# jameshensman/pyvb

Measured on AMD Instinct MI355X. Metric: VB update iterations/sec (T=10k, D=64, N=1024 LDS); ELBO rel-err vs NumPy, higher is better.
Workload: dtype f64; 1 GPU; LDS T=10000 D=64 K=64, 1024 replicates per GPU (BASELINE configs[2]); replicates_total=1024, parallelism=replicates sharded over 1 GPU(s), collective=none (1 GPU), degraded=False

## Files before the change

### pyvb_amd/csrc/k_sweep.hip

```cpp
#include "common.h"

struct SweepArgs {
    const double* Xold; double* Xnew; const double* Y; const double* gains; const int* warm;
    const double *A_mean, *C_mean;
    const double *QA, *RC;
    double* trash;
    double* U;
    double* Sxx;
    int N, T, D, K, dir;
    int W;
    const unsigned char* active;
    const int* len;
    int keep_x;
    Layout L;
};

#define MFMA(a, b, c) __builtin_amdgcn_mfma_f64_16x16x4f64((a), (b), (c), 0, 0, 0)

constexpr int BOUNDARY_BLOCK = 16;

template <int NP>
__device__ __forceinline__ double boundary_chain(double v, const double* M, size_t stride, size_t off, int n, const double* u) {
#pragma unroll
    for (int b = 0; b < NP; b += BOUNDARY_BLOCK) {
        if (b >= n) break;
        double m[BOUNDARY_BLOCK];
#pragma unroll
        for (int e = 0; e < BOUNDARY_BLOCK; ++e) m[e] = M[(size_t)(b + e < n ? b + e : n - 1) * stride + off];
#pragma unroll
        for (int e = 0; e < BOUNDARY_BLOCK; ++e) v += (b + e < n ? m[e] : 0.0) * u[b + e];
    }
    return v;
}

template <int DP, int KP>
__device__ __forceinline__ double boundary_update(bool first, const double* g, const Layout& L, const double* Am, const double* Cm,
                                                  int D, int K, int lane, double xn, const double* y, double* ux, double* uy, double* vs,
                                                  const double* QA = nullptr, const double* RC = nullptr) {
    const bool dense = QA != nullptr;
    const int lc = lane < D ? lane : D - 1, kc = lane < K ? lane : K - 1;
    const double qb = g[L.oqr + lc], rb = g[L.oqr + 64 + kc], yk = y[kc], w0 = g[L.ow0 + lc];
    ux[lane] = lane < D ? ((first && !dense) ? qb * xn : xn) : 0.0;
    uy[lane] = lane < K ? (dense ? yk : rb * yk) : 0.0;
    __syncthreads();
    double v = boundary_chain<DP>(first ? w0 : 0.0, dense ? QA : Am, first ? D : 1, (size_t)lc * (first ? 1 : D), D, ux);
    if (!first && !dense) v = qb * v;
    v = boundary_chain<KP>(v, dense ? RC : Cm, D, lc, K, uy);
    vs[lane] = lane < D ? v : 0.0;
    __syncthreads();
    const double s = boundary_chain<DP>(0.0, g + (first ? L.oS0 : L.oS2), L.DP, lc, D, vs);
    __syncthreads();
    return lane < D ? s : 0.0;
}

template <int DT, int KT, bool FULL, int MODE, bool SPLIT>
__global__ void __launch_bounds__(64) k_sweep(SweepArgs a) {
    constexpr int DS = 4 * DT, KS = 4 * KT, DP = 16 * DT, KP = 16 * KT;
    __shared__ double gl[MODE == 2 ? DP * 17 : DT * KS * 64];
    __shared__ double xs[64];
    __shared__ double vs[64], ux[64], uy[64];
    const int n = blockIdx.x, w = SPLIT ? blockIdx.y : 0, lane = threadIdx.x, c = lane & 15, q = lane >> 4;
    if (!a.active[n]) return;
    const int T = a.T, D = a.D, K = a.K;
    const int TL = a.len ? a.len[n] : T;
    const bool fwd = (a.dir == 0);
    const int sgn = fwd ? 1 : -1;
    const Layout& L = a.L;
    const double* g = a.gains + (size_t)n * L.gains_total;
    const double* Xo = a.Xold + (size_t)n * T * DP;
    double* Xn = a.Xnew + (size_t)n * T * DP;
    const double* Yn = a.Y + (size_t)n * T * K;

    double rn[DT][DS], ip[DT][DS];
    {
        const double* Rn = g + (fwd ? L.oFn : L.oBn);
        const double* Ip = g + (fwd ? L.oBn : L.oFn);
#pragma unroll
        for (int m = 0; m < DT; ++m)
#pragma unroll
            for (int s = 0; s < DS; ++s) {
                rn[m][s] = Rn[(m * DS + s) * 64 + lane];
                ip[m][s] = (MODE == 2) ? 0.0 : Ip[(m * DS + s) * 64 + lane];
            }
        if constexpr (MODE != 2) {
            const double* Gp = g + L.oGp;
            for (int i = 0; i < DT * KS; ++i) gl[i * 64 + lane] = Gp[i * 64 + lane];
        }
    }

    const int Tint = TL - 2;
    const int Lw = SPLIT ? split_part_len(T, a.W) : Tint;
    const int ow = SPLIT ? w * Lw : 0;
    const int Tw = (Tint - ow < Lw) ? Tint - ow : Lw;
    const int J = a.warm[n * 2 + a.dir];

    const int t_first = fwd ? 0 : TL - 1, t_last = fwd ? TL - 1 : 0;
    const double* Am = a.A_mean + (size_t)n * D * D;
    const double* Cm = a.C_mean + (size_t)n * K * D;
    const double* QAm = a.QA ? a.QA + (size_t)n * D * D : nullptr;
    const double* RCm = a.RC ? a.RC + (size_t)n * K * D : nullptr;
    if (!SPLIT || ow <= J) {
        const double* xo = Xo + (size_t)(t_first + sgn) * DP;
        const double s = boundary_update<DP, KP>(fwd, g, L, Am, Cm, D, K, lane, xo[xpos(lane < D ? lane : D - 1)],
                                                 Yn + (size_t)t_first * K, ux, uy, vs, QAm, RCm);
        if (w == 0 && lane < DP) Xn[(size_t)t_first * DP + xpos(lane)] = (lane < D) ? s : 0.0;
        xs[lane] = (lane < D) ? s : 0.0;
    }
    __builtin_amdgcn_fence(__ATOMIC_RELEASE, "workgroup");
    __builtin_amdgcn_s_barrier();
    __builtin_amdgcn_fence(__ATOMIC_ACQUIRE, "workgroup");

    if (Tw > 0) {
        const int Lseg = (Tw + 15) >> 4;
        const int cL = c * Lseg;
        const int before = ow + cL;
        const int jc = -(J < before ? J : before);
        const int jstart = -((J < ow + 15 * Lseg) ? J : ow + 15 * Lseg);
        d4 x[DT];
#pragma unroll
        for (int m = 0; m < DT; ++m)
#pragma unroll
            for (int r = 0; r < 4; ++r) x[m][r] = (jc == -before) ? xs[16 * m + 4 * r + q] : 0.0;

        const int tbase = fwd ? (1 + before) : (TL - 2 - before);
        const int tsafe = fwd ? 1 : TL - 2;
        auto active = [&](int j) { int tt = cL + j; return j >= jc && j < Lseg && tt < Tw; };
        d2 yv[KS / 2];
        d4 mo[DT];
        auto load_y = [&](int j, d2* dst) {
            const double* p = Yn + (size_t)(active(j) ? tbase + sgn * j : tsafe) * K;
#pragma unroll
            for (int i = 0; i < KS / 2; ++i) {
                const int d0 = 8 * i + 2 * q;
                if constexpr (FULL) {
                    dst[i] = *reinterpret_cast<const d2*>(p + d0);
                } else {
                    dst[i][0] = p[d0 < K ? d0 : K - 1];
                    dst[i][1] = p[d0 + 1 < K ? d0 + 1 : K - 1];
                }
            }
        };
        auto load_o = [&](int j, d4* dst) {
            const double* p = Xo + (size_t)((active(j) ? tbase + sgn * j : tsafe) + sgn) * DP;
#pragma unroll
            for (int m = 0; m < DT; ++m) dst[m] = *reinterpret_cast<const d4*>(p + (m * 4 + q) * 4);
        };
        auto store_x = [&](double* out) {
#pragma unroll
            for (int m = 0; m < DT; ++m) *reinterpret_cast<d4*>(out + (m * 4 + q) * 4) = x[m];
        };
        double* const trash = a.trash + (size_t)n * 256;
        double* out_pending = trash;
        double* const Un = a.U + (size_t)n * T * DP;
        auto u_row = [&](int j) { return (active(j) && j >= 0) ? Un + (size_t)(tbase + sgn * j) * DP : trash; };
        auto load_u = [&](int j, d4* dst) {
            const double* p = Un + (size_t)(active(j) ? tbase + sgn * j : tsafe) * DP;
#pragma unroll
            for (int m = 0; m < DT; ++m) dst[m] = *reinterpret_cast<const d4*>(p + (m * 4 + q) * 4);
        };
        auto select_tile = [&](int m, bool act, const d4* acc) {
#pragma unroll
            for (int r = 0; r < 4; ++r) x[m][r] = act ? acc[m][r] : x[m][r];
        };
        auto pending_row = [&](int j, bool act) {
            return (act && j >= 0 && (a.keep_x || before + j == Tint - 1)) ? Xn + (size_t)(tbase + sgn * j) * DP : trash;
        };
        auto finish_step = [&](int j, const d4* acc) {
            const bool act = active(j);
#pragma unroll
            for (int m = 0; m < DT; ++m) select_tile(m, act, acc);
            out_pending = pending_row(j, act);
        };
        auto mul_resident = [&](d4* acc, auto& M, const d4* v) {
#pragma unroll
            for (int s = 0; s < DS; ++s)
#pragma unroll
                for (int m = 0; m < DT; ++m) acc[m] = MFMA(M[m][s], v[s >> 2][s & 3], acc[m]);
        };
        if constexpr (MODE == 2) {
            constexpr int PF = 3;
            d4 ub[PF][DT];
            double* const tl = gl;
            for (int i = lane; i < DP * 17; i += 64) tl[i] = 0.0;
            d4 sxx[DT][DT];
#pragma unroll
            for (int m = 0; m < DT; ++m)
#pragma unroll
                for (int k = 0; k < DT; ++k) sxx[m][k] = d4{0.0, 0.0, 0.0, 0.0};
            auto tile_read = [&](double (*xt)[4]) {
#pragma unroll
                for (int m = 0; m < DT; ++m)
#pragma unroll
                    for (int s4 = 0; s4 < 4; ++s4) xt[m][s4] = tl[(16 * m + c) * 17 + 4 * s4 + q];
            };
            auto tile_accumulate = [&](double (*xt)[4]) {
#pragma unroll
                for (int s4 = 0; s4 < 4; ++s4)
#pragma unroll
                    for (int m = 0; m < DT; ++m)
#pragma unroll
                        for (int k = m; k < DT; ++k) sxx[m][k] = MFMA(xt[m][s4], xt[k][s4], sxx[m][k]);
            };
            auto tile_stage = [&](int m, bool keep) {
#pragma unroll
                for (int r = 0; r < 4; ++r) tl[(16 * m + 4 * r + q) * 17 + c] = keep ? x[m][r] : 0.0;
            };
#pragma unroll
            for (int p = 0; p < PF; ++p) { load_u(jstart + p, ub[p]); store_x(trash + 64 * p); }
            for (int j = jstart; j < Lseg; j += PF) {
#pragma unroll
                for (int p = 0; p < PF; ++p) {
                    d4 acc[DT];
                    double xt[DT][4];
                    tile_read(xt);
#pragma unroll
                    for (int m = 0; m < DT; ++m) acc[m] = ub[p][m];
                    __builtin_amdgcn_sched_barrier(0);
                    load_u(j + p + PF, ub[p]);
                    store_x(out_pending);
                    __builtin_amdgcn_sched_barrier(0);
                    mul_resident(acc, rn, x);
                    const bool act = active(j + p);
                    const bool keep = act && j + p >= 0;
                    tile_accumulate(xt);
                    finish_step(j + p, acc);
#pragma unroll
                    for (int m = 0; m < DT; ++m) tile_stage(m, keep);
                }
            }
            {
                double xt[DT][4];
                tile_read(xt);
                tile_accumulate(xt);
            }
            store_x(out_pending);
            double* Sn = a.Sxx + ((size_t)n * (SPLIT ? a.W : 1) + w) * DP * DP;
#pragma unroll
            for (int m = 0; m < DT; ++m)
#pragma unroll
                for (int k = m; k < DT; ++k)
#pragma unroll
                    for (int e = 0; e < 4; ++e) {
                        const int row = 16 * m + 4 * e + q, col = 16 * k + c;
                        Sn[(size_t)row * DP + col] = sxx[m][k][e];
                        if (k > m) Sn[(size_t)col * DP + row] = sxx[m][k][e];
                    }
        } else {
        load_y(jstart, yv);
        store_x(trash);
        if constexpr (MODE == 1) store_x(trash + 64);
        load_o(jstart, mo);
        for (int j = jstart; j < Lseg; ++j) {
            d4 acc[DT];
            {
#pragma unroll
                for (int m = 0; m < DT; ++m) acc[m] = d4{0.0, 0.0, 0.0, 0.0};
                int goff = lane;
                asm volatile("" : "+v"(goff));
#pragma unroll
                for (int s = 0; s < KS; ++s)
#pragma unroll
                    for (int m = 0; m < DT; ++m) acc[m] = MFMA(gl[(m * KS + s) * 64 + goff], yv[s >> 1][s & 1], acc[m]);
                __builtin_amdgcn_sched_barrier(0);
                load_y(j + 1, yv);
                store_x(out_pending);
                __builtin_amdgcn_sched_barrier(0);
            }
            mul_resident(acc, rn, x);
            {
                if constexpr (MODE == 1) {
                    __builtin_amdgcn_sched_barrier(0);
                    double* ur = u_row(j);
#pragma unroll
                    for (int m = 0; m < DT; ++m) *reinterpret_cast<d4*>(ur + (m * 4 + q) * 4) = acc[m];
                    __builtin_amdgcn_sched_barrier(0);
                }
                mul_resident(acc, ip, mo);
                __builtin_amdgcn_sched_barrier(0);
                load_o(j + 1, mo);
                __builtin_amdgcn_sched_barrier(0);
            }
            finish_step(j, acc);
        }
        store_x(out_pending);
        }
        const int clast = (Tw - 1) / Lseg;
        __builtin_amdgcn_s_barrier();
        if (c == clast) {
#pragma unroll
            for (int m = 0; m < DT; ++m)
#pragma unroll
                for (int r = 0; r < 4; ++r) xs[16 * m + 4 * r + q] = x[m][r];
        }
        __builtin_amdgcn_fence(__ATOMIC_RELEASE, "workgroup");
        __builtin_amdgcn_s_barrier();
        __builtin_amdgcn_fence(__ATOMIC_ACQUIRE, "workgroup");
    }

    if (!SPLIT || w == ((Tint > 0) ? (Tint - 1) / Lw : 0)) {
        const double s = boundary_update<DP, KP>(!fwd, g, L, Am, Cm, D, K, lane, xs[lane],
                                                 Yn + (size_t)t_last * K, ux, uy, vs, QAm, RCm);
        if (lane < DP) Xn[(size_t)t_last * DP + xpos(lane)] = (lane < D) ? s : 0.0;
    }
}

struct StepArgs {
    double* X; const double* Y; const double* gains; const double *A_mean, *C_mean, *QA, *RC;
    const unsigned char* active;
    const int* len;
    int N, T, D, K, t;
    Layout L;
};

__global__ void __launch_bounds__(64) k_step(StepArgs a) {
    const int n = blockIdx.x, lane = threadIdx.x;
    if (!a.active[n]) return;
    const int T = a.T, D = a.D, K = a.K, t = a.t, DP = a.L.DP;
    const int TL = a.len ? a.len[n] : T;
    if (t >= TL) return;
    const Layout& L = a.L;
    const double* g = a.gains + (size_t)n * L.gains_total;
    double* X = a.X + (size_t)n * T * DP;
    const double* y = a.Y + ((size_t)n * T + t) * K;
    const int cls = (t == 0) ? 0 : (t == TL - 1 ? 2 : 1);
    const int row = lane % DP;
    if (cls != 1) {
        __shared__ double vs[64], ux[64], uy[64];
        const double* nbr = X + (size_t)(cls == 0 ? 1 : TL - 2) * DP;
        const double s = boundary_update<64, 64>(cls == 0, g, L, a.A_mean + (size_t)n * D * D, a.C_mean + (size_t)n * K * D, D, K, lane,
                                                 nbr[xpos(lane < D ? lane : D - 1)], y, ux, uy, vs,
                                                 a.QA ? a.QA + (size_t)n * D * D : nullptr, a.RC ? a.RC + (size_t)n * K * D : nullptr);
        if (lane < DP) X[(size_t)t * DP + xpos(lane)] = (lane < D) ? s : 0.0;
        return;
    }
    const int DS = L.DS, KS = L.KS;
    double s = 0.0;
    for (int j = 0; j < D; ++j) s += g[L.oFn + pos_nat(row, j, DS)] * X[(size_t)(t - 1) * DP + xpos(j)];
    for (int j = 0; j < D; ++j) s += g[L.oBn + pos_nat(row, j, DS)] * X[(size_t)(t + 1) * DP + xpos(j)];
    for (int k = 0; k < K; ++k) s += g[L.oGp + pos_perm(row, k, KS)] * y[k];
    if (lane < DP) X[(size_t)t * DP + xpos(lane)] = (lane < D) ? s : 0.0;
}

template <int DT, int KT>
static int launch_sweep_t(pyvb_lds* h, const SweepArgs& a, bool read_cache) {
    const bool full = h->D == 16 * DT && a.K == 16 * KT;
    const int mode = a.dir == PYVB_FORWARD ? 1 : (read_cache ? 2 : 0);
#define PYVB_SWEEP_CASE(F, M) do { if (h->W > 1) hipLaunchKernelGGL((k_sweep<DT, KT, F, M, true>), dim3(h->N, h->W), dim3(64), 0, h->stream, a); \
                                   else hipLaunchKernelGGL((k_sweep<DT, KT, F, M, false>), dim3(h->N), dim3(64), 0, h->stream, a); } while (0)
    if (full) { if (mode == 1) PYVB_SWEEP_CASE(true, 1); else if (mode == 2) PYVB_SWEEP_CASE(true, 2); else PYVB_SWEEP_CASE(true, 0); }
    else { if (mode == 1) PYVB_SWEEP_CASE(false, 1); else if (mode == 2) PYVB_SWEEP_CASE(false, 2); else PYVB_SWEEP_CASE(false, 0); }
#undef PYVB_SWEEP_CASE
    return PYVB_OK;
}

int launch_sweep(pyvb_lds* h, int direction, int src, bool read_cache, bool keep_x) {
    if (h->big) return launch_sweep_big(h, direction, src, read_cache);
    SweepArgs a;
    a.keep_x = (keep_x || direction != PYVB_FORWARD) ? 1 : 0;
    a.W = h->W;
    a.Xold = h->X[src]; a.Xnew = h->X[1 - src]; a.Y = lds_sweep_Y(h); a.gains = h->gains; a.warm = h->warm;
    a.trash = h->trash; a.U = h->U; a.Sxx = h->sxx; a.A_mean = h->A_mean; a.C_mean = lds_sweep_C(h);
    a.QA = h->dense ? h->QA : nullptr; a.RC = h->dense ? h->RC : nullptr;
    a.N = h->N; a.T = h->T; a.D = h->D; a.K = lds_sweep_K(h); a.dir = direction; a.L = h->L; a.active = h->active; a.len = h->len;
    {
        TimedLaunch tl(h, direction == PYVB_FORWARD ? PYVB_K_SWEEP_FWD : PYVB_K_SWEEP_BWD);
        switch (h->L.DT * 10 + h->L.KT) {
            case 11: launch_sweep_t<1, 1>(h, a, read_cache); break;
            case 12: launch_sweep_t<1, 2>(h, a, read_cache); break;
            case 14: launch_sweep_t<1, 4>(h, a, read_cache); break;
            case 21: launch_sweep_t<2, 1>(h, a, read_cache); break;
            case 22: launch_sweep_t<2, 2>(h, a, read_cache); break;
            case 24: launch_sweep_t<2, 4>(h, a, read_cache); break;
            case 41: launch_sweep_t<4, 1>(h, a, read_cache); break;
            case 42: launch_sweep_t<4, 2>(h, a, read_cache); break;
            case 44: launch_sweep_t<4, 4>(h, a, read_cache); break;
            default: pyvb_set_error("unsupported tile shape"); return PYVB_E_ARG;
        }
    }
    HIPCHK(hipGetLastError());
    return PYVB_OK;
}

struct PermArgs { const double* src; double* dst; size_t rows; int D, DP, to_internal; };
__global__ void __launch_bounds__(256) k_permute(PermArgs a) {
    const int per = a.DP > 64 ? 128 : 64;
    const size_t row = (size_t)blockIdx.x * (256 / per) + (threadIdx.x / per);
    const int d = threadIdx.x % per;
    if (row >= a.rows || d >= a.DP) return;
    if (a.to_internal) a.dst[row * a.DP + xpos(d)] = (d < a.D) ? a.src[row * a.D + d] : 0.0;
    else if (d < a.D) a.dst[row * a.D + d] = a.src[row * a.DP + xpos(d)];
}

int launch_permute(pyvb_lds* h, const double* src, double* dst, int to_internal) {
    PermArgs a; a.src = src; a.dst = dst; a.rows = (size_t)h->N * h->T; a.D = h->D; a.DP = h->L.DP; a.to_internal = to_internal;
    const size_t per_block = a.DP > 64 ? 2 : 4;
    hipLaunchKernelGGL(k_permute, dim3((unsigned)((a.rows + per_block - 1) / per_block)), dim3(256), 0, h->stream, a);
    HIPCHK(hipGetLastError());
    return PYVB_OK;
}

struct CarryArgs { const double* src; double* dst; const unsigned char* active; size_t per; };
__global__ void __launch_bounds__(256) k_carry(CarryArgs a) {
    const int n = blockIdx.y;
    if (a.active[n]) return;
    const double* s = a.src + (size_t)n * a.per;
    double* d = a.dst + (size_t)n * a.per;
    for (size_t i = (size_t)blockIdx.x * 256 + threadIdx.x; i < a.per; i += (size_t)gridDim.x * 256) d[i] = s[i];
}

int launch_carry(pyvb_lds* h, const double* src, double* dst, size_t per) {
    CarryArgs a; a.src = src; a.dst = dst; a.active = h->active; a.per = per;
    const size_t blocks = (per + 255) / 256;
    hipLaunchKernelGGL(k_carry, dim3((unsigned)(blocks < 64 ? blocks : 64), h->N), dim3(256), 0, h->stream, a);
    HIPCHK(hipGetLastError());
    return PYVB_OK;
}

int launch_step(pyvb_lds* h, int t) {
    if (h->big) return launch_step_big(h, t);
    StepArgs a;
    a.X = h->X[h->st.cur]; a.Y = lds_sweep_Y(h); a.gains = h->gains; a.A_mean = h->A_mean; a.C_mean = lds_sweep_C(h);
    a.QA = h->dense ? h->QA : nullptr; a.RC = h->dense ? h->RC : nullptr;
    a.N = h->N; a.T = h->T; a.D = h->D; a.K = lds_sweep_K(h); a.t = t; a.L = h->L; a.active = h->active; a.len = h->len;
    TimedLaunch tl(h, PYVB_K_STEP);
    hipLaunchKernelGGL(k_step, dim3(h->N), dim3(64), 0, h->stream, a);
    HIPCHK(hipGetLastError());
    return PYVB_OK;
}
```

Measured before the change: 92.15 VB iterations/s per 1024 replicates (whole job).

## Replace forward-sweep warm-up with seam correction pass and specialize keep_x

```diff
diff --git a/pyvb_amd/csrc/k_sweep.hip b/pyvb_amd/csrc/k_sweep.hip
--- a/pyvb_amd/csrc/k_sweep.hip
+++ b/pyvb_amd/csrc/k_sweep.hip
@@ -1,4 +1,6 @@
+#include <type_traits>
 #include "common.h"
+#include "sweep_plan.h"
 
 struct SweepArgs {
     const double* Xold; double* Xnew; const double* Y; const double* gains; const int* warm;
@@ -53,7 +55,7 @@
     return lane < D ? s : 0.0;
 }
 
-template <int DT, int KT, bool FULL, int MODE, bool SPLIT>
+template <int DT, int KT, bool FULL, int MODE, bool SPLIT, bool KEEPX = true>
 __global__ void __launch_bounds__(64) k_sweep(SweepArgs a) {
     constexpr int DS = 4 * DT, KS = 4 * KT, DP = 16 * DT, KP = 16 * KT;
     __shared__ double gl[MODE == 2 ? DP * 17 : DT * KS * 64];
@@ -88,11 +90,12 @@
         }
     }
 
-    const int Tint = TL - 2;
+    const int J = a.warm[n * 2 + a.dir];
+    const SweepPart part = sweep_part(TL, T, SPLIT ? a.W : 1, w, J, MODE == 1 && fwd);
+    const int Tint = part.Tint;
     const int Lw = SPLIT ? split_part_len(T, a.W) : Tint;
-    const int ow = SPLIT ? w * Lw : 0;
-    const int Tw = (Tint - ow < Lw) ? Tint - ow : Lw;
-    const int J = a.warm[n * 2 + a.dir];
+    const int ow = part.ow;
+    const int Tw = part.Tw;
 
     const int t_first = fwd ? 0 : TL - 1, t_last = fwd ? TL - 1 : 0;
     const double* Am = a.A_mean + (size_t)n * D * D;
@@ -111,20 +114,19 @@
     __builtin_amdgcn_fence(__ATOMIC_ACQUIRE, "workgroup");
 
     if (Tw > 0) {
-        const int Lseg = (Tw + 15) >> 4;
-        const int cL = c * Lseg;
-        const int before = ow + cL;
-        const int jc = -(J < before ? J : before);
-        const int jstart = -((J < ow + 15 * Lseg) ? J : ow + 15 * Lseg);
+        const int Lseg = part.Lseg;
+        const SweepColumn col = sweep_column(part, c);
+        const int before = col.before;
+        const int jstart = sweep_first_step(part);
         d4 x[DT];
 #pragma unroll
         for (int m = 0; m < DT; ++m)
 #pragma unroll
-            for (int r = 0; r < 4; ++r) x[m][r] = (jc == -before) ? xs[16 * m + 4 * r + q] : 0.0;
+            for (int r = 0; r < 4; ++r) x[m][r] = (col.kind == SWEEP_START_BOUNDARY) ? xs[16 * m + 4 * r + q] : 0.0;
 
         const int tbase = fwd ? (1 + before) : (TL - 2 - before);
         const int tsafe = fwd ? 1 : TL - 2;
-        auto active = [&](int j) { int tt = cL + j; return j >= jc && j < Lseg && tt < Tw; };
+        auto active = [&](int j) { return sweep_active(part, col, j); };
         d2 yv[KS / 2];
         d4 mo[DT];
         auto load_y = [&](int j, d2* dst) {
@@ -163,7 +165,7 @@
             for (int r = 0; r < 4; ++r) x[m][r] = act ? acc[m][r] : x[m][r];
         };
         auto pending_row = [&](int j, bool act) {
-            return (act && j >= 0 && (a.keep_x || before + j == Tint - 1)) ? Xn + (size_t)(tbase + sgn * j) * DP : trash;
+            return (act && j >= 0 && (KEEPX || before + j == Tint - 1)) ? Xn + (size_t)(tbase + sgn * j) * DP : trash;
         };
         auto finish_step = [&](int j, const d4* acc) {
             const bool act = active(j);
@@ -207,26 +209,35 @@
             };
 #pragma unroll
             for (int p = 0; p < PF; ++p) { load_u(jstart + p, ub[p]); store_x(trash + 64 * p); }
-            for (int j = jstart; j < Lseg; j += PF) {
-#pragma unroll
-                for (int p = 0; p < PF; ++p) {
-                    d4 acc[DT];
-                    double xt[DT][4];
-                    tile_read(xt);
-#pragma unroll
-                    for (int m = 0; m < DT; ++m) acc[m] = ub[p][m];
-                    __builtin_amdgcn_sched_barrier(0);
-                    load_u(j + p + PF, ub[p]);
-                    store_x(out_pending);
-                    __builtin_amdgcn_sched_barrier(0);
-                    mul_resident(acc, rn, x);
-                    const bool act = active(j + p);
-                    const bool keep = act && j + p >= 0;
-                    tile_accumulate(xt);
-                    finish_step(j + p, acc);
+            auto step = [&](int j, int p, d4* ubp, auto counted) {
+                constexpr bool COUNTED = decltype(counted)::value;
+                d4 acc[DT];
+                double xt[DT][4];
+                if constexpr (COUNTED) tile_read(xt);
+#pragma unroll
+                for (int m = 0; m < DT; ++m) acc[m] = ubp[m];
+                __builtin_amdgcn_sched_barrier(0);
+                load_u(j + p + PF, ubp);
+                store_x(out_pending);
+                __builtin_amdgcn_sched_barrier(0);
+                mul_resident(acc, rn, x);
+                const bool act = active(j + p);
+                [[maybe_unused]] const bool keep = act && j + p >= 0;
+                if constexpr (COUNTED) tile_accumulate(xt);
+                finish_step(j + p, acc);
+                if constexpr (COUNTED) {
 #pragma unroll
                     for (int m = 0; m < DT; ++m) tile_stage(m, keep);
                 }
+            };
+            int j = jstart;
+            for (; j + PF <= 0; j += PF) {
+#pragma unroll
+                for (int p = 0; p < PF; ++p) step(j, p, ub[p], std::false_type{});
+            }
+            for (; j < Lseg; j += PF) {
+#pragma unroll
+                for (int p = 0; p < PF; ++p) step(j, p, ub[p], std::true_type{});
             }
             {
                 double xt[DT][4];
@@ -247,7 +258,7 @@
                     }
         } else {
         load_y(jstart, yv);
-        store_x(trash);
+        if constexpr (KEEPX) store_x(trash);
         if constexpr (MODE == 1) store_x(trash + 64);
         load_o(jstart, mo);
         for (int j = jstart; j < Lseg; ++j) {
@@ -263,7 +274,7 @@
                     for (int m = 0; m < DT; ++m) acc[m] = MFMA(gl[(m * KS + s) * 64 + goff], yv[s >> 1][s & 1], acc[m]);
                 __builtin_amdgcn_sched_barrier(0);
                 load_y(j + 1, yv);
-                store_x(out_pending);
+                if constexpr (KEEPX) store_x(out_pending);
                 __builtin_amdgcn_sched_barrier(0);
             }
             mul_resident(acc, rn, x);
@@ -282,7 +293,8 @@
             }
             finish_step(j, acc);
         }
-        store_x(out_pending);
+        if constexpr (KEEPX) store_x(out_pending);
+        else store_x((col.count > 0 && before + col.count == Tint) ? Xn + (size_t)(tbase + sgn * (col.count - 1)) * DP : trash);
         }
         const int clast = (Tw - 1) / Lseg;
         __builtin_amdgcn_s_barrier();
@@ -295,6 +307,58 @@
         __builtin_amdgcn_fence(__ATOMIC_RELEASE, "workgroup");
         __builtin_amdgcn_s_barrier();
         __builtin_amdgcn_fence(__ATOMIC_ACQUIRE, "workgroup");
+        if constexpr (MODE == 1 && !SPLIT) {
+            const int ncorr = sweep_correction_steps(part);
+            if (ncorr > 0) {
+                const bool seam = col.kind == SWEEP_START_SEAM;
+                d4 dl[DT];
+#pragma unroll
+                for (int m = 0; m < DT; ++m)
+#pragma unroll
+                    for (int r = 0; r < 4; ++r) {
+                        const double e = __shfl_up(x[m][r], 1, 16);
+                        dl[m][r] = seam ? e : 0.0;
+                    }
+                auto correct = [&](auto keep) {
+                    constexpr bool KEEP = decltype(keep)::value;
+                    auto c_row = [&](int k) { return seam ? Un + (size_t)(tbase + k) * DP : trash; };
+                    auto x_row = [&](int k) { return (seam && before + k != Tint - 1) ? Xn + (size_t)(tbase + k) * DP : trash + 64; };
+                    auto load_row = [&](const double* p, d4* dst) {
+#pragma unroll
+                        for (int m = 0; m < DT; ++m) dst[m] = *reinterpret_cast<const d4*>(p + (m * 4 + q) * 4);
+                    };
+                    auto store_row = [&](double* p, const d4* src) {
+#pragma unroll
+                        for (int m = 0; m < DT; ++m) *reinterpret_cast<d4*>(p + (m * 4 + q) * 4) = src[m];
+                    };
+                    d4 cb[DT], xb[DT];
+                    load_row(c_row(0), cb);
+                    if constexpr (KEEP) load_row(x_row(0), xb);
+                    store_row(trash + 128, dl);
+                    if constexpr (KEEP) store_row(trash + 192, dl);
+                    for (int k = 0; k < ncorr; ++k) {
+                        d4 acc[DT], cs[DT], xc[DT];
+#pragma unroll
+                        for (int m = 0; m < DT; ++m) acc[m] = d4{0.0, 0.0, 0.0, 0.0};
+                        mul_resident(acc, rn, dl);
+#pragma unroll
+                        for (int m = 0; m < DT; ++m) {
+                            dl[m] = acc[m];
+                            cs[m] = cb[m] + acc[m];
+                            if constexpr (KEEP) xc[m] = xb[m] + acc[m];
+                        }
+                        const int kn = k + 1 < ncorr ? k + 1 : k;
+                        __builtin_amdgcn_sched_barrier(0);
+                        load_row(c_row(kn), cb);
+                        if constexpr (KEEP) load_row(x_row(kn), xb);
+                        store_row(c_row(k), cs);
+                        if constexpr (KEEP) store_row(x_row(k), xc);
+                        __builtin_amdgcn_sched_barrier(0);
+                    }
+                };
+                correct(std::integral_constant<bool, KEEPX>{});
+            }
+        }
     }
 
     if (!SPLIT || w == ((Tint > 0) ? (Tint - 1) / Lw : 0)) {
@@ -345,10 +409,12 @@
 static int launch_sweep_t(pyvb_lds* h, const SweepArgs& a, bool read_cache) {
     const bool full = h->D == 16 * DT && a.K == 16 * KT;
     const int mode = a.dir == PYVB_FORWARD ? 1 : (read_cache ? 2 : 0);
-#define PYVB_SWEEP_CASE(F, M) do { if (h->W > 1) hipLaunchKernelGGL((k_sweep<DT, KT, F, M, true>), dim3(h->N, h->W), dim3(64), 0, h->stream, a); \
-                                   else hipLaunchKernelGGL((k_sweep<DT, KT, F, M, false>), dim3(h->N), dim3(64), 0, h->stream, a); } while (0)
-    if (full) { if (mode == 1) PYVB_SWEEP_CASE(true, 1); else if (mode == 2) PYVB_SWEEP_CASE(true, 2); else PYVB_SWEEP_CASE(true, 0); }
-    else { if (mode == 1) PYVB_SWEEP_CASE(false, 1); else if (mode == 2) PYVB_SWEEP_CASE(false, 2); else PYVB_SWEEP_CASE(false, 0); }
+#define PYVB_SWEEP_CASE(F, M, X) do { if (h->W > 1) hipLaunchKernelGGL((k_sweep<DT, KT, F, M, true, X>), dim3(h->N, h->W), dim3(64), 0, h->stream, a); \
+                                      else hipLaunchKernelGGL((k_sweep<DT, KT, F, M, false, X>), dim3(h->N), dim3(64), 0, h->stream, a); } while (0)
+#define PYVB_SWEEP_FORWARD(F) do { if (a.keep_x) PYVB_SWEEP_CASE(F, 1, true); else PYVB_SWEEP_CASE(F, 1, false); } while (0)
+    if (full) { if (mode == 1) PYVB_SWEEP_FORWARD(true); else if (mode == 2) PYVB_SWEEP_CASE(true, 2, true); else PYVB_SWEEP_CASE(true, 0, true); }
+    else { if (mode == 1) PYVB_SWEEP_FORWARD(false); else if (mode == 2) PYVB_SWEEP_CASE(false, 2, true); else PYVB_SWEEP_CASE(false, 0, true); }
+#undef PYVB_SWEEP_FORWARD
 #undef PYVB_SWEEP_CASE
     return PYVB_OK;
 }
diff --git a/pyvb_amd/csrc/sweep_plan.h b/pyvb_amd/csrc/sweep_plan.h
--- /dev/null
+++ b/pyvb_amd/csrc/sweep_plan.h
@@ -0,0 +1,74 @@
+#pragma once
+#include "geometry.h"
+
+enum { SWEEP_START_BOUNDARY = 0, SWEEP_START_SEAM = 1, SWEEP_START_WARM = 2 };
+enum { SWEEP_COLUMNS = 16 };
+
+struct SweepPart {
+    int Tint;
+    int ow;
+    int Tw;
+    int Lseg;
+    int J;
+    bool seams;
+};
+
+struct SweepColumn {
+    int before;
+    int count;
+    int jc;
+    int kind;
+};
+
+PYVB_HD static inline SweepPart sweep_part(int TL, int T, int W, int w, int J, bool forward) {
+    SweepPart p;
+    p.Tint = TL - 2;
+    const int Lw = W > 1 ? split_part_len(T, W) : p.Tint;
+    p.ow = W > 1 ? w * Lw : 0;
+    p.Tw = (p.Tint - p.ow < Lw) ? p.Tint - p.ow : Lw;
+    p.Lseg = p.Tw > 0 ? (p.Tw + 15) >> 4 : 0;
+    p.J = J;
+    p.seams = forward && W == 1;
+    return p;
+}
+
+PYVB_HD static inline int sweep_column_count(const SweepPart& p, int c) {
+    const int left = p.Tw - c * p.Lseg;
+    return left <= 0 ? 0 : (left < p.Lseg ? left : p.Lseg);
+}
+
+PYVB_HD static inline SweepColumn sweep_column(const SweepPart& p, int c) {
+    SweepColumn s;
+    s.before = p.ow + c * p.Lseg;
+    s.count = sweep_column_count(p, c);
+    if (s.before <= p.J) { s.kind = SWEEP_START_BOUNDARY; s.jc = -s.before; }
+    else if (p.seams && c > 0 && s.count >= p.J && sweep_column_count(p, c - 1) >= p.J) { s.kind = SWEEP_START_SEAM; s.jc = 0; }
+    else { s.kind = SWEEP_START_WARM; s.jc = -p.J; }
+    return s;
+}
+
+PYVB_HD static inline void sweep_seam_columns(const SweepPart& p, int& c0, int& c1) {
+    c0 = 1; c1 = 0;
+    if (!p.seams || p.Tw < p.J || p.Lseg < p.J || p.Lseg <= 0) return;
+    c0 = p.Lseg > p.J ? 1 : 2;
+    c1 = (p.Tw - p.J) / p.Lseg;
+    c1 = c1 < SWEEP_COLUMNS - 1 ? c1 : SWEEP_COLUMNS - 1;
+}
+
+PYVB_HD static inline int sweep_first_step(const SweepPart& p) {
+    int c0, c1;
+    sweep_seam_columns(p, c0, c1);
+    const int last = p.ow + (SWEEP_COLUMNS - 1) * p.Lseg;
+    if (c0 > c1) return -(p.J < last ? p.J : last);
+    return (c0 > 1 || c1 < SWEEP_COLUMNS - 1) ? -p.J : 0;
+}
+
+PYVB_HD static inline int sweep_correction_steps(const SweepPart& p) {
+    int c0, c1;
+    sweep_seam_columns(p, c0, c1);
+    return c0 <= c1 ? p.J : 0;
+}
+
+PYVB_HD static inline bool sweep_active(const SweepPart& p, const SweepColumn& s, int j) {
+    return j >= s.jc && j < p.Lseg && (s.before - p.ow) + j < p.Tw;
+}
```

Result: faster. 93.72 VB iterations/s per 1024 replicates (whole job) (median of 6 runs) (+1.7%).
